# eloimoliner/BABE

Measured on AMD Instinct MI355X. Metric: audio-sec/s (blind BWE, 10 s @ 44.1 kHz clips, 35 EDM steps 2nd order), whole job, higher is better.
Workload: dtype f32

## Files before the change

### babe_amd/_cabi.py

```python
import ctypes as C


class ConvArgs(C.Structure):
    _fields_ = [
        ("in_", C.c_void_p), ("in_bs", C.c_long), ("in_cs", C.c_long),
        ("in2", C.c_void_p), ("in2_bs", C.c_long), ("in2_cs", C.c_long), ("cin_split", C.c_int),
        ("w_packed", C.c_void_p),
        ("out", C.c_void_p), ("out_bs", C.c_long), ("out_cs", C.c_long),
        ("res", C.c_void_p), ("res_bs", C.c_long), ("res_cs", C.c_long),
        ("in_scale", C.c_void_p), ("oscale", C.c_void_p),
        ("alpha", C.c_float), ("rbeta", C.c_float),
        ("B", C.c_int), ("Cin", C.c_int), ("Cout", C.c_int), ("F", C.c_int), ("T", C.c_int),
        ("KH", C.c_int), ("KW", C.c_int), ("dil", C.c_int),
        ("stat_mode", C.c_int), ("stat_cg", C.c_int), ("stat_x", C.c_void_p), ("stat_scale", C.c_void_p), ("stat_part", C.c_void_p),
        ("fbias", C.c_void_p),
    ]


class WgradArgs(C.Structure):
    _fields_ = [("x", C.c_void_p), ("x_bs", C.c_long), ("x_cs", C.c_long),
                ("x2", C.c_void_p), ("x2_bs", C.c_long), ("x2_cs", C.c_long), ("cin_split", C.c_int),
                ("g", C.c_void_p), ("g_bs", C.c_long), ("g_cs", C.c_long),
                ("B", C.c_int), ("Cin", C.c_int), ("Cout", C.c_int), ("F", C.c_int), ("T", C.c_int),
                ("KH", C.c_int), ("KW", C.c_int), ("dil", C.c_int)]
# ... 25 lines not shown
                ("oct", C.c_void_p), ("binoct", C.c_void_p), ("tw4096", C.c_void_p),
                ("nocts", C.c_int), ("binsoct", C.c_int), ("coef", C.c_void_p * 8),
                ("wg_first", C.c_void_p), ("wg_count", C.c_void_p), ("nwg", C.c_int),
                ("wg_rec", C.c_void_p), ("band_rec", C.c_void_p), ("abl", C.c_int),
                ("max_wg_count", C.c_int), ("min_log2T", C.c_int), ("max_log2T", C.c_int),
                ("sum_T", C.c_long), ("sum_M", C.c_long), ("sum_TlogT", C.c_double),
                ("kdeg", C.c_int), ("kpoly", C.c_float * 12)]


class FitCfg(C.Structure):
    _fields_ = [("mu_fc", C.c_float), ("mu_A", C.c_float), ("tol_fc", C.c_float), ("tol_A", C.c_float),
                ("fcmin", C.c_float), ("fcmax", C.c_float), ("Amin", C.c_float), ("Amax", C.c_float),
                ("max_iter", C.c_int), ("clamp_fc", C.c_int), ("clamp_A", C.c_int), ("only_negative_A", C.c_int),
                ("weighting", C.c_int), ("kernel", C.c_int)]


class EvalDesc(C.Structure):
    _fields_ = [("unet_plan", C.c_void_p), ("unet_state", C.c_void_p), ("cqt_plan", C.c_void_p), ("L", C.c_int),
                ("rff_freq", C.c_void_p), ("rff_n", C.c_int),
                ("emb_W", C.c_void_p * 3), ("emb_b", C.c_void_p * 3), ("emb_dim", C.c_int * 4),
                ("film_W", C.c_void_p), ("film_b", C.c_void_p), ("film_J", C.c_int),
                ("nfft", C.c_int), ("fs", C.c_float), ("env_inv", C.c_void_p), ("tw4096", C.c_void_p), ("K", C.c_int),
                ("fit", FitCfg), ("blind", C.c_int), ("shared", C.c_int), ("hpf", C.c_int),
                ("xi", C.c_float), ("score_mode", C.c_int), ("audio_len_norm", C.c_float)]


class DnConvArgs(C.Structure):
    _fields_ = [("in_", C.c_void_p), ("in_bs", C.c_long), ("in_cs", C.c_long), ("IH", C.c_int), ("IW", C.c_int),
                ("bias", C.c_void_p),
                ("out", C.c_void_p), ("out_bs", C.c_long), ("out_cs", C.c_long), ("out_H", C.c_int), ("out_W", C.c_int),
                ("out_hstep", C.c_int), ("out_h0", C.c_int), ("out_wstep", C.c_int), ("out_w0", C.c_int),
                ("res", C.c_void_p), ("res_bs", C.c_long), ("res_cs", C.c_long),
                ("B", C.c_int), ("Cin", C.c_int), ("Cout", C.c_int), ("OH", C.c_int), ("OW", C.c_int),
                ("KH", C.c_int), ("KW", C.c_int), ("stride", C.c_int), ("pad_t", C.c_int), ("pad_l", C.c_int),
                ("pad_mode", C.c_int), ("act", C.c_int), ("ksplit", C.c_int), ("ws", C.c_void_p)]


STRUCTS = {"babe_conv_args": ConvArgs, "babe_wgrad_args": WgradArgs, "babe_packed_conv": CPackedConv, "babe_unet_block": CBlock,
           "babe_unet_plan_desc": CPlanDesc, "babe_cqt_bands": CqtBands, "babe_fit_cfg": FitCfg, "babe_eval_desc": EvalDesc,
           "babe_dnconv_args": DnConvArgs}

_P, _L, _I, _F, _D, _S = C.c_void_p, C.c_long, C.c_int, C.c_float, C.c_double, C.c_char_p

SIGS = {
    "babe_version": (_S, []),
    "babe_last_error": (_S, []),
    "babe_conv2d_wino85_stat_slots": (_I, [C.POINTER(ConvArgs)]),
    "babe_conv_packed_size": (_L, [_I, _I, _I, _I, _I]),
    "babe_conv_pack_weights_nt": (_I, [_P, _P, _I, _I, _I, _I, _I, _I, _P]),
    "babe_conv_pack_weights_bf16": (_I, [_P, _P, _I, _I, _I, _I, _I, _I, _P]),
    "babe_conv_packed_size_bf16": (_L, [_I, _I, _I, _I, _I, _I]),
    "babe_units_size": (_L, [_I, _I, _I]),
    "babe_scale_gelu_units": (_I, [_P, _P, _P, _I, _I, _I, _I, _P]),
    "babe_conv2d_bf16_units_supported": (_I, [C.POINTER(ConvArgs)]),
    "babe_conv2d_bf16_units": (_I, [C.POINTER(ConvArgs), _P, _P]),
    "babe_conv2d_wino_supported": (_I, [C.POINTER(ConvArgs)]),
    "babe_conv_pack_weights_wino": (_I, [_P, _P, _I, _I, _I, _I, _I, _P]),
    "babe_conv_packed_size_wino": (_L, [_I, _I, _I, _I]),
    "babe_conv2d_wino4_supported": (_I, [C.POINTER(ConvArgs)]),
    "babe_conv_pack_weights_wino4": (_I, [_P, _P, _I, _I, _I, _I, _I, _P]),
    "babe_conv_packed_size_wino4": (_L, [_I, _I, _I, _I]),
    "babe_conv2d_wino45": (_I, [C.POINTER(ConvArgs), _P, _P]),
    "babe_conv2d_wino45_supported": (_I, [C.POINTER(ConvArgs)]),
    "babe_conv_pack_weights_wino45": (_I, [_P, _P, _I, _I, _I, _I, _I, _P]),
    "babe_conv_packed_size_wino45": (_L, [_I, _I, _I]),
    "babe_prof_nslots": (_I, []),
    "babe_prof_slot_name": (_S, [_I]),
    "babe_prof_enable": (_I, [_I]),
    "babe_prof_conv_slot": (_I, [_I]),
    "babe_prof_read": (_I, [_P, _P, _P, _P, _P]),
    "babe_prof_dispatch_counts": (_I, [_P, _I]),
    "babe_prof_timeline": (_L, [_P, _P, _P, _P, _P, _L]),
    "babe_prof_pending": (_L, []),
    "babe_gn_partial": (_I, [_P, _P, _I, _I, _L, _I, _P]),
    "babe_gn_stats": (_I, [_P, _P, _P, _P, _P, _L, _P, _P, _I, _I, _I, _L, _I, _F, _P]),
    "babe_gn_finalize": (_I, [_P, _P, _P, _L, _P, _P, _I, _I, _I, _L, _I, _F, _P]),
    "babe_scale_gelu_fin": (_I, [_P, _P, _P, _P, _L, _P, _P, _P, _I, _I, _I, _L, _I, _F, _P]),
    "babe_scale_gelu": (_I, [_P, _P, _P, _I, _I, _L, _P]),
    "babe_gn_bwd_partial": (_I, [_P, _P, _P, _P, _I, _I, _I, _L, _I, _P]),
    "babe_gn_bwd_apply": (_I, [_P, _P, _P, _P, _P, _P, _P, _F, _I, _I, _I, _L, _I, _F, _P]),
    "babe_gn_bwd_apply_merge": (_I, [_P, _P, _P, _P, _P, _P, _P, _F, _I, _I, _I, _L, _I, _F, _P, _P, _F, _F]),
    "babe_gn_bwd_partial_nogelu": (_I, [_P, _P, _P, _P, _I, _I, _I, _L, _I, _P]),
    "babe_gn_bwd_apply_nogelu": (_I, [_P, _P, _P, _P, _P, _P, _P, _F, _I, _I, _I, _L, _I, _F, _P]),
    "babe_resample": (_I, [_P, _L, _L, _P, _L, _L, _I, _I, _I, _I, _I, _F, _F, _P]),
    "babe_resample_res": (_I, [_P, _L, _L, _P, _L, _L, _P, _L, _L, _I, _I, _I, _I, _I, _F, _F, _P]),
    "babe_resample_sinc": (_I, [_P, _L, _P, _L, _I, _L, _L, _P, _P, _I, _I, _I, _P]),
    "babe_resample_sinc_adjoint": (_I, [_P, _L, _P, _L, _I, _L, _L, _P, _P, _I, _I, _I, _P]),
    "babe_iir_workspace": (_L, [_I, _L, _I]),
    "babe_iir_filter": (_I, [_P, _L, _P, _L, _I, _L, _P, _P, _I, _I, _I, _P, _L, _P, _L, _P]),
    "babe_decimate": (_I, [_P, _L, _P, _L, _I, _L, _L, _I, _I, _P]),
    "babe_clip_residual": (_I, [_P, _L, _P, _L, _F, _P, _L, _P, _L, _P, _I, _I, _L, _P]),
    "babe_clip_fwd": (_I, [_P, _L, _F, _P, _L, _I, _L, _P]),
    "babe_clip_adj": (_I, [_P, _L, _P, _L, _P, _L, _I, _L, _P]),
    "babe_specnorm_workspace": (_L, [_I, _I, _I]),
    "babe_specnorm_seed": (_I, [_P, _L, _I, _I, _I, _P, _L, _I, _P, _L, _P]),
    "babe_stft_mag_workspace": (_L, [_I, _I, _I]),
    "babe_stft_mag_fwd": (_I, [_P, _L, _L, _P, _I, _I, _P, _P, _I, _I, _P, _P]),
    "babe_stft_mag_vjp": (_I, [_P, _P, _P, _I, _I, _P, _L, _L, _I, _I, _P, _P, _L, _P]),
    "babe_conv_packed_size_wino85": (_L, [_I, _I, _I]),
    "babe_conv_pack_weights_wino85": (_I, [_P, _P, _I, _I, _I, _I, _I, _P]),
    "babe_conv2d_wino85_supported": (_I, [C.POINTER(ConvArgs)]),
    "babe_conv2d_wino85_preferred": (_I, [C.POINTER(ConvArgs)]),
    "babe_conv2d_wino85": (_I, [C.POINTER(ConvArgs), _P, _P]),
    "babe_conv2d_wino85_set_waves": (_I, [_I]),
    "babe_conv2d_auto": (_I, [C.POINTER(ConvArgs), C.POINTER(CPackedConv), _I, _P]),
    "babe_unet_plan_create": (_P, [C.POINTER(CPlanDesc)]),
    "babe_unet_plan_destroy": (None, [_P]),
    "babe_unet_state_create": (_P, []),
    "babe_unet_state_destroy": (None, [_P]),
    "babe_unet_workspace_bytes": (_L, [_P, _I, C.POINTER(_I)]),
    "babe_unet_fwd": (_I, [_P, _P, C.POINTER(_P), _P, _L, _I, C.POINTER(_I), _P, _L, C.POINTER(_P), _P]),
    "babe_unet_vjp": (_I, [_P, _P, C.POINTER(_P), C.POINTER(_P), _P]),
    "babe_axpby4d": (_I, [_P, _L, _L, _P, _L, _L, _I, _I, _I, _I, _F, _F, _P]),
    "babe_axpby2_4d": (_I, [_P, _L, _L, _P, _L, _L, _P, _L, _L, _I, _I, _I, _I, _F, _F, _P]),
    "babe_linear": (_I, [_P, _P, _P, _P, _I, _I, _I, _I, _P]),
    "babe_rff": (_I, [_P, _P, _P, _I, _I, _P]),
    "babe_rfft_mixed": (_I, [_P, _P, _P, _P, _P, _I, _I, _I, _I, _P, _I, _P, _I, _P, _P, _P, _I, _P]),
    "babe_fft_twiddle_transpose": (_I, [_P, _P, _P, _I, _I, _I, _I, _P]),
    "babe_cqt_band_analysis": (_I, [C.POINTER(CqtBands), _P, _P, _I, _P]),
    "babe_cqt_band_synthesis": (_I, [C.POINTER(CqtBands), _P, _P, _L, _I, _P]),
    "babe_cqt_gather": (_I, [_P, _L, _P, _P, _P, _P, _I, _I, _F, _P, _I, _P]),
    "babe_spec_scale": (_I, [_P, _P, _P, _P, _I, _I, _F, _F, _I, _P]),
    "babe_cqt_design_create": (_P, [_D, _I, _I, _I, _D]),
    "babe_cqt_design_destroy": (None, [_P]),
    "babe_cqt_design_get": (_L, [_P, _S, _P, _L]),
    "babe_cqt_plan_create": (_P, [_D, _I, _I, _I, _D]),
    "babe_cqt_plan_destroy": (None, [_P]),
    "babe_cqt_workspace_bytes": (_L, [_P, _I]),
    "babe_cqt_fwd": (_I, [_P, _P, _P, _P, _I, _P]),
    "babe_cqt_bwd": (_I, [_P, _P, _P, _P, _I, _P]),
    "babe_cqt_fwd_adjoint": (_I, [_P, _P, _P, _P, _I, _P]),
    "babe_cqt_bwd_adjoint": (_I, [_P, _P, _P, _P, _I, _P]),
    "babe_cqt_hpf": (_I, [_P, _P, _P, _P, _I, _P]),
    "babe_stft_fwd": (_I, [_P, _L, _I, _P, _P, _I, _I, _I, _P, _P]),
    "babe_spec_filter_istft": (_I, [_P, _P, _L, _P, _I, _I, _I, _P, _P]),
    "babe_ola": (_I, [_P, _P, _P, _L, _P, _L, _P, _I, _I, _I, _I, _I, _P]),
    "babe_residual_seed": (_I, [_P, _L, _P, _I, _P, _P, _L, _I, _I, _P]),
    "babe_stft_mag_stats": (_I, [_P, _P, _P, _I, _I, _I, _I, _P]),
    "babe_design_filter": (_I, [_P, _P, _I, _I, _I, _F, _I, _P]),
    "babe_filter_fit": (_I, [_P, _P, _P, _I, _I, _I, _F, _I, C.POINTER(FitCfg), _P]),
    "babe_filter_loss_grad": (_I, [_P, _L, _P, _P, _I, _I, _I, _F, _I, C.POINTER(FitCfg), _P]),
    "babe_fir_same": (_I, [_P, _L, _P, _I, _P, _L, _I, _I, _I, _P]),
    "babe_fir_sqerr_fwd": (_I, [_P, _L, _P, _L, _P, _I, _P, _P, _I, _I, _P]),
    "babe_fir_sqerr_bwd": (_I, [_P, _L, _P, _P, _I, _P, _I, _I, _P]),
    "babe_plane_bin_energy": (_I, [_P, _P, _I, _I, _I, _P]),
    "babe_lsd_num_frames": (_L, [_I, _I, _I]),
    "babe_lsd_frames": (_I, [_P, _L, _P, _L, _I, _I, _I, _I, _I, _I, _F, _P, _P, _P]),
    "babe_lincomb3": (_I, [_P, _F, _P, _F, _P, _F, _P, _L, _P]),
    "babe_add_obs_noise": (_I, [_P, _L, _P, _L, _F, _I, _L, _P]),
    "babe_mask_blend": (_I, [_P, _P, _L, _P, _P, _I, _L, _P]),
    "babe_sumsq_partial": (_I, [_P, _L, _P, _I, _I, _L, _P]),
    "babe_stft_dist_partial": (_I, [_P, _P, _P, _P, _I, _I, _I, _I, _I, _P]),
    "babe_stft_dist_grad": (_I, [_P, _P, _P, _P, _I, _P, _I, _I, _I, _I, _I, _P]),
    "babe_cos_partial": (_I, [_P, _L, _P, _L, _P, _I, _I, _L, _P]),
    "babe_residual_seed_alt": (_I, [_P, _L, _P, _L, _P, _I, _P, _P, _L, _I, _I, _I, _F, _P]),
    "babe_score_direction": (_I, [_P, _P, _P, _P, _I, _P, _F, _F, _F, _I, _I, _I, _L, _P]),
    "babe_eval_workspace_bytes": (_L, [C.POINTER(EvalDesc), _I]),
    "babe_score_eval": (_I, [C.POINTER(EvalDesc), _P, _F, _F, _F, _F, _F, _P, _P, _P, _P, _P, _P, _P, _L, _I, _P]),
    "babe_dn_conv2d": (_I, [C.POINTER(DnConvArgs), _P, _P]),
    "babe_dn_pack_weights": (_I, [_P, _P, _I, _I, _I, _I, _I, _I, _I, _P]),
    "babe_dn_packed_size": (_L, [_I, _I, _I, _I]),
    "babe_dn_upsample_add": (_I, [_P, _L, _L, _P, _L, _L, _I, _I, _I, _I, _I, _I, _I, _I, _P]),
    "babe_dn_sam_gate": (_I, [_P, _P, _P, _L, _L, _P, _L, _L, _I, _I, _L, _P]),
    "babe_dn_fill_input": (_I, [_P, _P, _P, _I, _I, _I, _I, _P]),
    "babe_dn_stft": (_I, [_P, _L, _I, _P, _I, _I, _I, _I, _P, _P]),
    "babe_dn_istft": (_I, [_P, _P, _P, _L, _I, _I, _I, _I, _I, _P, _P]),
# ... 38 lines not shown
```

### babe_amd/csrc/norm.hip

```cpp
#include "common.h"
#include "../../include/babe_hip.h"
#include "prof.h"
#include "gelu.h"
#include <cstdlib>

namespace {

using babe_gelu::gelu_f;
using babe_gelu::gelu_grad_f;

__device__ __forceinline__ void block_reduce2(double& s0, double& s1, double* sh) {
    s0 = wave_sum(s0);
    s1 = wave_sum(s1);
    const int lane = threadIdx.x & 63, wave = threadIdx.x >> 6;
    if (lane == 0) {
        sh[wave * 2] = s0;
        sh[wave * 2 + 1] = s1;
    }
    __syncthreads();
    if (threadIdx.x == 0) {
        double a = 0, b = 0;
        for (int w = 0; w < (int)(blockDim.x >> 6); ++w) {
            a += sh[w * 2];
            b += sh[w * 2 + 1];
// ... 292 lines not shown
                const float4 x0 = *reinterpret_cast<const float4*>(x + base + i);
                const float4 d0 = *reinterpret_cast<const float4*>(dadu + base + i);
                const float4 x1 = *reinterpret_cast<const float4*>(x + base + i + st);
                const float4 d1 = *reinterpret_cast<const float4*>(dadu + base + i + st);
                sc_sum += term(x0, d0);
                sc_sum += term(x1, d1);
            }
            for (; i < hi; i += st)
                sc_sum += term(*reinterpret_cast<const float4*>(x + base + i), *reinterpret_cast<const float4*>(dadu + base + i));
            s0 += (double)sc * sc_sum;
        }
    }
    block_reduce2(s0, s1, sh);
    if (threadIdx.x == 0) part[(long)bg * S + s] = s0;
}

template <bool GELU>
__global__ __launch_bounds__(256) void gn_bwd_apply_kernel(const float* __restrict__ x, const float* __restrict__ da,
                                                           const float* __restrict__ gy,
                                                           const float* __restrict__ scale,
                                                           const float* __restrict__ stats,
                                                           const double* __restrict__ part, float* __restrict__ gx,
                                                           float rbeta, int C, int G, long hw, int S, float eps,
                                                           const float* __restrict__ acc, float ca, float cb) {
    const int c = blockIdx.y, b = blockIdx.z;
    const int cg = C / G;
    const int g = c / cg;
    const long n = (long)cg * hw;
    __shared__ double S1_sh;
    if (threadIdx.x < 64) {
        double v = 0;
        for (int s = threadIdx.x; s < S; s += 64) v += part[(long)(b * G + g) * S + s];
        v = wave_sum(v);
        if (threadIdx.x == 0) S1_sh = v;
    }
    __syncthreads();
    const double S1 = S1_sh;
    const float mean = stats[(b * G + g) * 3 + 0];
    const float sd = stats[(b * G + g) * 3 + 1];
    const double se = (double)sd + eps;
    const float coef = (sd > 0.f) ? (float)(S1 * se / ((double)(n - 1) * sd * se * se)) : 0.f;
    const float sc = scale[b * C + c];
    const long base = ((long)b * C + c) * hw;
    const long nv = hw / 4;
    const float4* x4 = reinterpret_cast<const float4*>(x + base);
    const float4* d4 = reinterpret_cast<const float4*>(da + base);
    const float4* g4 = gy ? reinterpret_cast<const float4*>(gy + base) : nullptr;
    float4* o4 = reinterpret_cast<float4*>(gx + base);
    for (long i = (long)blockIdx.x * blockDim.x + threadIdx.x; i < nv; i += (long)gridDim.x * blockDim.x) {
        const float4 xv = x4[i];
        float4 dv = d4[i];
        if (GELU) {
            dv.x *= gelu_grad_f(xv.x * sc);
            dv.y *= gelu_grad_f(xv.y * sc);
            dv.z *= gelu_grad_f(xv.z * sc);
            dv.w *= gelu_grad_f(xv.w * sc);
        }
        float4 o;
        o.x = sc * dv.x - (xv.x - mean) * coef;
        o.y = sc * dv.y - (xv.y - mean) * coef;
        o.z = sc * dv.z - (xv.z - mean) * coef;
        o.w = sc * dv.w - (xv.w - mean) * coef;
        if (g4) {
            const float4 gv = g4[i];
            o.x += rbeta * gv.x;
            o.y += rbeta * gv.y;
            o.z += rbeta * gv.z;
            o.w += rbeta * gv.w;
        }
        if (acc) {
#pragma clang fp contract(off)
            const float4 av = reinterpret_cast<const float4*>(acc + base)[i];
            const float px = ca * av.x, py = ca * av.y, pz = ca * av.z, pw = ca * av.w;
            const float qx = cb * o.x, qy = cb * o.y, qz = cb * o.z, qw = cb * o.w;
            o.x = px + qx;
            o.y = py + qy;
            o.z = pz + qz;
            o.w = pw + qw;
        }
        o4[i] = o;
    }
}

}

static int abl_gn() {
    static const int v = [] { const char* e = getenv("BABE_ABL_GN"); return e ? atoi(e) : 0; }();
    return v;
}

extern "C" int babe_gn_partial(const float* x, double* part, int B, int G, long n, int S, void* stream) {
    BABE_CHECK_ARG(x && part && B > 0 && G > 0 && n > 1 && S > 0, "gn_partial: bad arguments");
    if (abl_gn() & 1) return BABE_OK;
    BABE_CHECK_ARG(n % 4 == 0, "gn_partial: group size %ld not a multiple of 4", n);
    BabeProfScope prof(BABE_SLOT_GN_STATS, 4.0 * B * G * (double)n, 0, 0, stream);
    hipLaunchKernelGGL(gn_partial_kernel<false>, dim3(S, B * G), dim3(256), 0, (hipStream_t)stream, x, part, n, S,
                       (int*)nullptr, (const float*)nullptr, (const float*)nullptr, 0L, (float*)nullptr, (float*)nullptr, 0, 1, 0.f);
    BABE_LAUNCH_CHECK();
    return BABE_OK;
}

extern "C" int babe_gn_stats(const float* x, double* part, int* ticket, const float* gamma, const float* film, long film_bs,
                             float* stats, float* scale, int B, int C, int G, long n, int S, float eps, void* stream) {
    BABE_CHECK_ARG(x && part && ticket && gamma && film && stats && scale && B > 0 && G > 0 && n > 1 && S > 0, "gn_stats: bad arguments");
    BABE_CHECK_ARG(n % 4 == 0 && G <= 64 && C % G == 0, "gn_stats: n=%ld C=%d G=%d unsupported", n, C, G);
    BabeProfScope prof(BABE_SLOT_GN_STATS, 4.0 * B * G * (double)n, 0, 0, stream);
    hipLaunchKernelGGL(gn_partial_kernel<true>, dim3(S, B * G), dim3(256), 0, (hipStream_t)stream, x, part, n, S, ticket, gamma,
                       film, film_bs, stats, scale, C, G, eps);
    BABE_LAUNCH_CHECK();
    return BABE_OK;
}

extern "C" int babe_gn_finalize(const double* part, const float* gamma, const float* film, long film_bs, float* stats,
                                float* scale, int B, int C, int G, long n, int S, float eps, void* stream) {
    BABE_CHECK_ARG(part && gamma && film && stats && scale, "gn_finalize: null pointer");
    BABE_CHECK_ARG(G <= 64 && C % G == 0, "gn_finalize: C=%d G=%d unsupported", C, G);
    BabeProfScope prof(BABE_SLOT_GN_STATS, 0, 0, 0, stream);
    hipLaunchKernelGGL(gn_finalize_kernel, dim3(B), dim3(256), 0, (hipStream_t)stream, part, gamma, film, film_bs,
                       stats, scale, C, G, n, S, eps);
    BABE_LAUNCH_CHECK();
    return BABE_OK;
}

extern "C" int babe_scale_gelu(const float* x, const float* scale, float* a, int B, int C, long hw, void* stream) {
    BABE_CHECK_ARG(x && scale && a && B > 0 && C > 0 && hw > 0, "scale_gelu: bad arguments");
    BABE_CHECK_ARG(hw % 4 == 0, "scale_gelu: plane size %ld not a multiple of 4", hw);
    BabeProfScope prof(BABE_SLOT_SCALE_GELU, 8.0 * B * C * (double)hw, 0, 0, stream);
    int bx = cdiv(hw / 4, 256 * 4);
    if (bx < 1) bx = 1;
    if (bx > 64) bx = 64;
    hipLaunchKernelGGL(scale_gelu_kernel, dim3(bx, C, B), dim3(256), 0, (hipStream_t)stream, x, scale, a, C, hw);
    BABE_LAUNCH_CHECK();
    return BABE_OK;
}

extern "C" int babe_scale_gelu_fin(const float* x, const double* part, const float* gamma, const float* film, long film_bs,
                                   float* stats, float* scale, float* a, int B, int C, int G, long hw, int S, float eps,
                                   void* stream) {
    BABE_CHECK_ARG(x && part && gamma && film && stats && scale && a && B > 0 && C > 0 && hw > 0 && S > 0, "scale_gelu_fin: bad arguments");
    BABE_CHECK_ARG(hw % 4 == 0 && G <= 64 && C % G == 0, "scale_gelu_fin: hw=%ld C=%d G=%d unsupported", hw, C, G);
    BabeProfScope prof(BABE_SLOT_SCALE_GELU, 8.0 * B * C * (double)hw, 0, 0, stream);
    int bx = cdiv(hw / 4, 256 * 4);
    if (bx < 1) bx = 1;
    if (bx > 64) bx = 64;
    const long n = (long)(C / G) * hw;
    hipLaunchKernelGGL(scale_gelu_fin_kernel, dim3(bx, C, B), dim3(256), 0, (hipStream_t)stream, x, part, gamma, film, film_bs,
                       stats, scale, a, C, G, hw, n, S, eps);
    BABE_LAUNCH_CHECK();
    return BABE_OK;
}

extern "C" long babe_units_size(int C, int F, int T) { return (long)(C / 8) * F * 4 * (T / 4 + 1); }

extern "C" int babe_scale_gelu_units(const float* x, const float* scale, void* au, int B, int C, int F, int T,
                                     void* stream) {
    BABE_CHECK_ARG(x && scale && au && B > 0 && C > 0 && F > 0 && T > 0, "scale_gelu_units: bad arguments");
    BABE_CHECK_ARG(T % 4 == 0 && C % 8 == 0, "scale_gelu_units: T=%d C=%d unsupported (need T %% 4 == 0, C %% 8 == 0)", T, C);
    BABE_CHECK_ARG(((uintptr_t)x & 15) == 0 && ((uintptr_t)au & 15) == 0, "scale_gelu_units: unaligned pointer");
    BabeProfScope prof(BABE_SLOT_SCALE_GELU, 6.0 * B * C * (double)F * T, 0, 0, stream);
    int bx = cdiv((long)F * (T / 4), 256 * 2);
    if (bx < 1) bx = 1;
    if (bx > 256) bx = 256;
    hipLaunchKernelGGL(scale_gelu_units_kernel, dim3(bx, C / 8, B), dim3(256), 0, (hipStream_t)stream, x, scale,
                       (bf16x8_n*)au, C, F, T);
    BABE_LAUNCH_CHECK();
    return BABE_OK;
}

extern "C" int babe_gn_bwd_partial(const float* x, const float* da, const float* scale, double* part, int B, int C,
                                   int G, long hw, int S, void* stream) {
    BABE_CHECK_ARG(x && da && scale && part, "gn_bwd_partial: null pointer");
    BABE_CHECK_ARG(hw % 4 == 0 && C % G == 0, "gn_bwd_partial: hw=%ld C=%d G=%d unsupported", hw, C, G);
    if (abl_gn() & 2) return BABE_OK;
    BabeProfScope prof(BABE_SLOT_GN_BWD_PARTIAL, 8.0 * B * C * (double)hw, 0, 0, stream);
    hipLaunchKernelGGL(gn_bwd_partial_kernel<true>, dim3(S, B * G), dim3(256), 0, (hipStream_t)stream, x, da, scale,
                       part, C, G, hw, S);
    BABE_LAUNCH_CHECK();
    return BABE_OK;
}

extern "C" int babe_gn_bwd_partial_nogelu(const float* x, const float* da, const float* scale, double* part, int B, int C,
                                          int G, long hw, int S, void* stream) {
    BABE_CHECK_ARG(x && da && scale && part, "gn_bwd_partial_nogelu: null pointer");
    BABE_CHECK_ARG(hw % 4 == 0 && C % G == 0, "gn_bwd_partial_nogelu: hw=%ld C=%d G=%d unsupported", hw, C, G);
    BabeProfScope prof(BABE_SLOT_GN_BWD_PARTIAL, 8.0 * B * C * (double)hw, 0, 0, stream);
    hipLaunchKernelGGL(gn_bwd_partial_kernel<false>, dim3(S, B * G), dim3(256), 0, (hipStream_t)stream, x, da, scale,
                       part, C, G, hw, S);
    BABE_LAUNCH_CHECK();
    return BABE_OK;
}

static int gn_bwd_apply_launch(bool gelu, const float* acc, float ca, float cb, const float* x, const float* da, const float* gy, const float* scale,
                                 const float* stats, const double* part, float* gx, float rbeta, int B, int C, int G,
                                 long hw, int S, float eps, void* stream) {
    BABE_CHECK_ARG(x && da && scale && stats && part && gx, "gn_bwd_apply: null pointer");
    BABE_CHECK_ARG(hw % 4 == 0 && C % G == 0, "gn_bwd_apply: hw=%ld C=%d G=%d unsupported", hw, C, G);
    BabeProfScope prof(BABE_SLOT_GN_BWD_APPLY, ((gy ? 16.0 : 12.0) + (acc ? 4.0 : 0.0)) * B * C * (double)hw, 0, 0, stream);
    int bx = cdiv(hw / 4, 256 * 4);
    if (bx < 1) bx = 1;
    if (bx > 64) bx = 64;
    if (gelu)
        hipLaunchKernelGGL(gn_bwd_apply_kernel<true>, dim3(bx, C, B), dim3(256), 0, (hipStream_t)stream, x, da, gy, scale, stats,
                           part, gx, rbeta, C, G, hw, S, eps, acc, ca, cb);
    else
        hipLaunchKernelGGL(gn_bwd_apply_kernel<false>, dim3(bx, C, B), dim3(256), 0, (hipStream_t)stream, x, da, gy, scale, stats,
                           part, gx, rbeta, C, G, hw, S, eps, acc, ca, cb);
    BABE_LAUNCH_CHECK();
    return BABE_OK;
}

extern "C" int babe_gn_bwd_apply(const float* x, const float* da, const float* gy, const float* scale,
                                 const float* stats, const double* part, float* gx, float rbeta, int B, int C, int G,
                                 long hw, int S, float eps, void* stream) {
    return gn_bwd_apply_launch(true, nullptr, 0.f, 0.f, x, da, gy, scale, stats, part, gx, rbeta, B, C, G, hw, S, eps, stream);
}

extern "C" int babe_gn_bwd_apply_nogelu(const float* x, const float* da, const float* gy, const float* scale,
                                        const float* stats, const double* part, float* gx, float rbeta, int B, int C, int G,
                                        long hw, int S, float eps, void* stream) {
    return gn_bwd_apply_launch(false, nullptr, 0.f, 0.f, x, da, gy, scale, stats, part, gx, rbeta, B, C, G, hw, S, eps, stream);
}

extern "C" int babe_gn_bwd_apply_merge(const float* x, const float* da, const float* gy, const float* scale,
                                 const float* stats, const double* part, float* gx, float rbeta, int B, int C, int G,
                                 long hw, int S, float eps, void* stream, const float* acc, float ca, float cb) {
    BABE_CHECK_ARG(acc && ((uintptr_t)acc & 15) == 0, "gn_bwd_apply_merge: acc must be a 16-byte aligned dense tensor");
    return gn_bwd_apply_launch(true, acc, ca, cb, x, da, gy, scale, stats, part, gx, rbeta, B, C, G, hw, S, eps, stream);
}
```

### include/babe_hip.h

```cpp
#ifndef BABE_HIP_H
#define BABE_HIP_H
#ifdef __cplusplus
extern "C" {
#endif

const char* babe_version(void);
const char* babe_last_error(void);

typedef struct { float* p; long bs; long cs; } babe_view;

typedef struct {
    const float* in;  long in_bs,  in_cs;
    const float* in2; long in2_bs, in2_cs; int cin_split;
    const float* w_packed;
    float* out;       long out_bs, out_cs;
    const float* res; long res_bs, res_cs;
    const float* in_scale;
    const float* oscale;
    float alpha, rbeta;
    int B, Cin, Cout, F, T, KH, KW, dil;
    int stat_mode, stat_cg;
    const float* stat_x; const float* stat_scale; double* stat_part;
    const float* fbias;
} babe_conv_args;
int babe_conv2d_wino85_stat_slots(const babe_conv_args* a);
int babe_conv2d(const babe_conv_args* a, void* stream);
int babe_conv_pack_weights(const float* w, float* dst, int Cout, int Cin, int KH, int KW,
                           int transpose_flip, void* stream);
long babe_conv_packed_size(int Cout, int Cin, int KH, int KW, int transpose_flip);
int babe_conv2d_nt(const babe_conv_args* a, int nt, void* stream);
int babe_conv_pack_weights_nt(const float* w, float* dst, int Cout, int Cin, int KH, int KW, int transpose_flip, int nt,
                              void* stream);
int babe_conv2d_bf16(const babe_conv_args* a, const void* w_bf16, int splits, void* stream);
int babe_conv_pack_weights_bf16(const float* w, void* dst, int Cout, int Cin, int KH, int KW, int transpose_flip,
                                int splits, void* stream);
long babe_conv_packed_size_bf16(int Cout, int Cin, int KH, int KW, int transpose_flip, int splits);
long babe_units_size(int C, int F, int T);
int babe_scale_gelu_units(const float* x, const float* scale, void* units, int B, int C, int F, int T, void* stream);
int babe_conv2d_bf16_units_supported(const babe_conv_args* a);
int babe_conv2d_bf16_units(const babe_conv_args* a, const void* w_bf16, void* stream);
int babe_conv2d_wino(const babe_conv_args* a, const float* w_wino, void* stream);
int babe_conv2d_wino_supported(const babe_conv_args* a);
int babe_conv_pack_weights_wino(const float* w, float* dst, int Cout, int Cin, int KH, int KW, int transpose_flip,
                                void* stream);
long babe_conv_packed_size_wino(int Cout, int Cin, int KH, int transpose_flip);
int babe_conv2d_wino4(const babe_conv_args* a, const float* w_wino4, void* stream);
int babe_conv2d_wino4_supported(const babe_conv_args* a);
int babe_conv_pack_weights_wino4(const float* w, float* dst, int Cout, int Cin, int KH, int KW, int transpose_flip,
                                 void* stream);
long babe_conv_packed_size_wino4(int Cout, int Cin, int KH, int transpose_flip);
int babe_conv2d_wino45(const babe_conv_args* a, const float* w_wino45, void* stream);
int babe_conv2d_wino45_supported(const babe_conv_args* a);
int babe_conv2d_wino45_preferred(const babe_conv_args* a);
int babe_conv_pack_weights_wino45(const float* w, float* dst, int Cout, int Cin, int KH, int KW, int transpose_flip,
                                  void* stream);
long babe_conv_packed_size_wino45(int Cout, int Cin, int transpose_flip);
int babe_conv2d_fewco(const babe_conv_args* a, const float* w, int transpose_flip, void* stream);
int babe_conv2d_fewco_supported(const babe_conv_args* a);
int babe_prof_nslots(void);
const char* babe_prof_slot_name(int slot);
int babe_prof_enable(int on);
int babe_prof_conv_slot(int slot);
int babe_prof_read(double* ms, double* bytes, double* flops, double* exec_flops, long* launches);
int babe_prof_dispatch_counts(long* counts, int reset);
long babe_prof_timeline(double* t0_ms, double* t1_ms, int* slot, int* lane, double* flops, long cap);
long babe_prof_pending(void);

int babe_gn_partial(const float* x, double* part, int B, int G, long n_per_group, int S, void* stream);
int babe_gn_stats(const float* x, double* part, int* ticket, const float* gamma, const float* film, long film_bs,
                  float* stats, float* scale, int B, int C, int G, long n_per_group, int S, float eps, void* stream);
int babe_gn_finalize(const double* part, const float* gamma, const float* film, long film_bs,
                     float* stats, float* scale, int B, int C, int G, long n_per_group, int S,
                     float eps, void* stream);
int babe_scale_gelu_fin(const float* x, const double* part, const float* gamma, const float* film, long film_bs, float* stats,
                        float* scale, float* a, int B, int C, int G, long hw, int S, float eps, void* stream);
int babe_scale_gelu(const float* x, const float* scale, float* a, int B, int C, long hw, void* stream);
int babe_gn_bwd_partial(const float* x, const float* da, const float* scale, double* part,
                        int B, int C, int G, long hw, int S, void* stream);
int babe_gn_bwd_apply(const float* x, const float* da, const float* gy, const float* scale,
                      const float* stats, const double* part, float* gx, float rbeta,
                      int B, int C, int G, long hw, int S, float eps, void* stream);
int babe_gn_bwd_apply_merge(const float* x, const float* da, const float* gy, const float* scale,
                            const float* stats, const double* part, float* gx, float rbeta,
                            int B, int C, int G, long hw, int S, float eps, void* stream,
                            const float* acc, float ca, float cb);
int babe_gn_bwd_partial_nogelu(const float* x, const float* da, const float* scale, double* part, int B, int C, int G, long hw,
                               int S, void* stream);
int babe_gn_bwd_apply_nogelu(const float* x, const float* da, const float* gy, const float* scale, const float* stats,
                             const double* part, float* gx, float rbeta, int B, int C, int G, long hw, int S, float eps,
                             void* stream);

int babe_resample(const float* in, long in_bs, long in_cs, float* out, long out_bs, long out_cs,
                  int B, int C, int F, int T, int mode, float alpha, float beta, void* stream);
int babe_resample_res(const float* in, long in_bs, long in_cs, const float* res, long res_bs, long res_cs, float* out,
                      long out_bs, long out_cs, int B, int C, int F, int T, int mode, float alpha, float beta, void* stream);

int babe_resample_sinc(const float* x, long x_bs, float* out, long out_bs, int B, long L_in, long L_out, const float* kernel,
                       const int* krange, int orig, int new_, int width, void* stream);
int babe_resample_sinc_adjoint(const float* g, long g_bs, float* out, long out_bs, int B, long L_in, long L_out,
                               const float* kernel, const int* krange, int orig, int new_, int width, void* stream);

long babe_iir_workspace(int B, long L, int order);
int babe_iir_filter(const float* x, long x_bs, float* y, long y_bs, int B, long L, const float* b, const float* a, int order,
                    int clamp, int adjoint, unsigned char* mask, long mask_bs, void* workspace, long workspace_bytes, void* stream);
int babe_decimate(const float* in, long in_bs, float* out, long out_bs, int B, long L_full, long L_dec, int factor, int adjoint,
                  void* stream);

int babe_clip_residual(const float* x, long x_bs, const float* y, long y_bs, float c, float* r, long r_bs, unsigned char* mask,
                       long mask_bs, double* part, int nblk, int B, long L, void* stream);
int babe_clip_fwd(const float* x, long x_bs, float c, float* out, long out_bs, int B, long L, void* stream);
int babe_clip_adj(const float* g, long g_bs, const unsigned char* mask, long mask_bs, float* out, long out_bs, int B, long L,
                  void* stream);
long babe_specnorm_workspace(int B, int rows, int cols);
int babe_specnorm_seed(const float* r, long r_bs, int rows, int cols, int iters, float* out, long out_bs, int B, void* workspace,
                       long workspace_bytes, void* stream);
long babe_stft_mag_workspace(int B, int frames, int win);
int babe_stft_mag_fwd(const float* x, long x_bs, long L, const float* window, int win, int hop, float* spec, float* mag, int B,
                      int frames, const float* tw4096, void* stream);
int babe_stft_mag_vjp(const float* G, const float* spec, const float* window, int win, int hop, float* gx, long gx_bs, long L,
                      int B, int frames, const float* tw4096, void* workspace, long workspace_bytes, void* stream);

long babe_conv_packed_size_wino85(int Cout, int Cin, int transpose_flip);
int babe_conv_pack_weights_wino85(const float* w, float* dst, int Cout, int Cin, int KH, int KW, int transpose_flip, void* stream);
int babe_conv2d_wino85_supported(const babe_conv_args* a);
int babe_conv2d_wino85_preferred(const babe_conv_args* a);
int babe_conv2d_wino85(const babe_conv_args* a, const float* w_wino85, void* stream);
int babe_conv2d_wino85_set_waves(int waves);

typedef struct {
    int Cout, Cin, KH, KW, nt, splits;
    const void *fwd, *bwd;
    const float *fwd_wino, *bwd_wino, *fwd_wino4, *bwd_wino4, *fwd_wino45, *bwd_wino45;
    const float* w_raw;
    const float *fwd_wino85, *bwd_wino85;
} babe_packed_conv;
int babe_conv2d_auto(babe_conv_args* a, const babe_packed_conv* pc, int transpose, void* stream);
typedef struct {
    int N, nd, k53;
    babe_packed_conv proj_in, res_conv, proj_out, H[8];
    const float* gamma[8];
    int film_aff[8], film_gate[8];
    const float *fb_proj_in, *fb_res_conv;
} babe_unet_block;
typedef struct {
    int nocts, bpo;
    int Ns[8];
    babe_unet_block init_blk[8], main_blk[8], up_out[8], up_blk[8], mid_blk, mid_out;
    babe_packed_conv pyr_conv[8];
} babe_unet_plan_desc;
void* babe_unet_plan_create(const babe_unet_plan_desc* desc);
void babe_unet_plan_destroy(void* plan);
void* babe_unet_state_create(void);
void babe_unet_state_destroy(void* state);
long babe_unet_workspace_bytes(const void* plan, int B, const int* T_oct);
int babe_unet_fwd(const void* plan, void* state, const float* const* C_in, const float* film, long film_bs, int B,
                  const int* T_oct, void* workspace, long workspace_bytes, float* const* outs, void* stream);
int babe_unet_vjp(const void* plan, void* state, const float* const* gouts, float* const* gC, void* stream);

int babe_axpby4d(const float* in, long in_bs, long in_cs, float* out, long out_bs, long out_cs,
                 int B, int C, int F, int T, float alpha, float beta, void* stream);
int babe_fill4d(float* out, long out_bs, long out_cs, int B, int C, int F, int T, float value, void* stream);
int babe_axpby2_4d(const float* x, long x_bs, long x_cs, const float* y, long y_bs, long y_cs, float* out, long out_bs,
                   long out_cs, int B, int C, int F, int T, float alpha, float beta, void* stream);

int babe_linear(const float* x, const float* W, const float* bias, float* out, int B, int K, int J,
                int relu, void* stream);
int babe_rff(const float* cnoise, const float* freq, float* out, int B, int R, void* stream);

int babe_rfft_mixed(const float* x_in, float* spec_out, const float* spec_in, float* x_out, float* work, int B, int N1,
                    int N2, int K2, const int* rad1, int nrad1, const int* rad2, int nrad2, const float* w1, const float* w2,
                    const float* tw, int direction, void* stream);
int babe_fft_twiddle_transpose(const float* in, float* out, const float* tw, int B, int N1, int N2,
                               int adjoint, void* stream);
// ... 192 lines not shown
```

Before: 2.470.

## Add alternate GroupNorm kernel forms with load rings and specialized apply variants

```diff
diff --git a/babe_amd/_cabi.py b/babe_amd/_cabi.py
--- a/babe_amd/_cabi.py
+++ b/babe_amd/_cabi.py
@@ -131,6 +131,8 @@
     "babe_gn_bwd_apply_merge": (_I, [_P, _P, _P, _P, _P, _P, _P, _F, _I, _I, _I, _L, _I, _F, _P, _P, _F, _F]),
     "babe_gn_bwd_partial_nogelu": (_I, [_P, _P, _P, _P, _I, _I, _I, _L, _I, _P]),
     "babe_gn_bwd_apply_nogelu": (_I, [_P, _P, _P, _P, _P, _P, _P, _F, _I, _I, _I, _L, _I, _F, _P]),
+    "babe_norm_set_form": (_I, [_I]),
+    "babe_norm_get_form": (_I, []),
     "babe_resample": (_I, [_P, _L, _L, _P, _L, _L, _I, _I, _I, _I, _I, _F, _F, _P]),
     "babe_resample_res": (_I, [_P, _L, _L, _P, _L, _L, _P, _L, _L, _I, _I, _I, _I, _I, _F, _F, _P]),
     "babe_resample_sinc": (_I, [_P, _L, _P, _L, _I, _L, _L, _P, _P, _I, _I, _I, _P]),
diff --git a/babe_amd/csrc/norm.hip b/babe_amd/csrc/norm.hip
--- a/babe_amd/csrc/norm.hip
+++ b/babe_amd/csrc/norm.hip
@@ -398,7 +398,341 @@
     }
 }
 
-}
+namespace f1 {
+
+__device__ __forceinline__ double sum4(const float4 v) {
+#pragma clang fp contract(off)
+    return (((double)v.x + (double)v.y) + (double)v.z) + (double)v.w;
+}
+__device__ __forceinline__ double sq4(const float4 v) {
+#pragma clang fp contract(off)
+    double a = (double)v.y * (double)v.y;
+    a = __builtin_fma((double)v.x, (double)v.x, a);
+    a = __builtin_fma((double)v.z, (double)v.z, a);
+    return __builtin_fma((double)v.w, (double)v.w, a);
+}
+
+template <int NT, int PAIR>
+__device__ __forceinline__ void slot_sums(const double* __restrict__ pg, int S, double& t0, double& t1) {
+    t0 = 0;
+    t1 = 0;
+    for (int q = threadIdx.x; q < S; q += NT * 4) {
+        double a[4], c[4];
+#pragma unroll
+        for (int k = 0; k < 4; ++k) {
+            const int qq = q + NT * k < S ? q + NT * k : S - 1;
+            a[k] = pg[(long)qq * PAIR];
+            c[k] = PAIR == 2 ? pg[(long)qq * PAIR + PAIR - 1] : 0.0;
+        }
+#pragma unroll
+        for (int k = 0; k < 4; ++k)
+            if (q + NT * k < S) {
+                t0 += a[k];
+                if (PAIR == 2) t1 += c[k];
+            }
+    }
+}
+
+__global__ __launch_bounds__(256) void gn_partial_kernel(const float* __restrict__ x, double* __restrict__ part, long n, int S) {
+    __shared__ double sh[8];
+    const int s = blockIdx.x;
+    const long bg = blockIdx.y;
+    const long chunk = ((n / 4 + S - 1) / S) * 4;
+    const long beg = (long)s * chunk;
+    long end = beg + chunk;
+    if (end > n) end = n;
+    const float* p = x + bg * n;
+    double s0 = 0, s1 = 0;
+    if (beg < end) {
+#pragma clang fp contract(off)
+        const long nv = (end - beg) / 4;
+        const float4* p4 = reinterpret_cast<const float4*>(p + beg);
+        long i = threadIdx.x;
+        for (; i + 7 * 256L < nv; i += 8 * 256L) {
+            float4 v[8];
+#pragma unroll
+            for (int k = 0; k < 8; ++k) v[k] = p4[i + k * 256L];
+            s0 += ((sum4(v[0]) + sum4(v[1])) + sum4(v[2])) + sum4(v[3]);
+            s1 += ((sq4(v[0]) + sq4(v[1])) + sq4(v[2])) + sq4(v[3]);
+            s0 += ((sum4(v[4]) + sum4(v[5])) + sum4(v[6])) + sum4(v[7]);
+            s1 += ((sq4(v[4]) + sq4(v[5])) + sq4(v[6])) + sq4(v[7]);
+        }
+        for (; i + 3 * 256L < nv; i += 4 * 256L) {
+            const float4 v0 = p4[i], v1 = p4[i + 256L], v2 = p4[i + 2 * 256L], v3 = p4[i + 3 * 256L];
+            s0 += ((sum4(v0) + sum4(v1)) + sum4(v2)) + sum4(v3);
+            s1 += ((sq4(v0) + sq4(v1)) + sq4(v2)) + sq4(v3);
+        }
+        for (; i < nv; i += 256L) {
+            const float4 v = p4[i];
+            s0 += sum4(v);
+            s1 += sq4(v);
+        }
+        for (long j = beg + nv * 4 + threadIdx.x; j < end; j += 256L) {
+            const double v = p[j];
+            s0 += v;
+            s1 = __builtin_fma(v, v, s1);
+        }
+    }
+    block_reduce2(s0, s1, sh);
+    if (threadIdx.x == 0) {
+        part[(bg * S + s) * 2] = s0;
+        part[(bg * S + s) * 2 + 1] = s1;
+    }
+}
+
+__device__ __forceinline__ float4 scale_gelu4(float4 v, const float sc) {
+#pragma clang fp contract(off)
+    v.x = gelu_f(v.x * sc);
+    v.y = gelu_f(v.y * sc);
+    v.z = gelu_f(v.z * sc);
+    v.w = gelu_f(v.w * sc);
+    return v;
+}
+
+constexpr int kGeluLoads = 4;
+
+template <int NLD, typename L>
+struct Ring {
+    L buf[NLD];
+    template <typename Load>
+    __device__ __forceinline__ void first(long i0, long gs, long nv, Load&& load) {
+#pragma unroll
+        for (int d = 0; d < NLD; ++d) {
+            const long j = i0 + d * gs;
+            buf[d] = load(j < nv ? j : nv - 1);
+        }
+    }
+    template <typename Load, typename Use>
+    __device__ __forceinline__ void run(long i0, long gs, long nv, Load&& load, Use&& use) {
+        for (long i = i0; i < nv; i += NLD * gs) {
+#pragma unroll
+            for (int d = 0; d < NLD; ++d) {
+                const long j = i + d * gs;
+                if (j < nv) use(j, buf[d]);
+                if (j + NLD * gs < nv) buf[d] = load(j + NLD * gs);
+            }
+        }
+    }
+};
+
+__global__ __launch_bounds__(256) void scale_gelu_kernel(const float* __restrict__ x, const float* __restrict__ scale,
+                                                         float* __restrict__ a, int C, long hw) {
+    const int c = blockIdx.y, b = blockIdx.z;
+    const long base = ((long)b * C + c) * hw;
+    const long nv = hw / 4;
+    const float4* x4 = reinterpret_cast<const float4*>(x + base);
+    float4* a4 = reinterpret_cast<float4*>(a + base);
+    const long i0 = (long)blockIdx.x * 256 + threadIdx.x, gs = (long)gridDim.x * 256;
+    auto load = [&](long j) { return x4[j]; };
+    Ring<kGeluLoads, float4> ring;
+    ring.first(i0, gs, nv, load);
+    const float sc = scale[b * C + c];
+    ring.run(i0, gs, nv, load, [&](long j, const float4 v) { a4[j] = scale_gelu4(v, sc); });
+}
+
+__global__ __launch_bounds__(256) void scale_gelu_fin_kernel(const float* __restrict__ x, const double* __restrict__ part,
+                                                             const float* __restrict__ gamma, const float* __restrict__ film,
+                                                             long film_bs, float* __restrict__ stats, float* __restrict__ scale,
+                                                             float* __restrict__ a, int C, int G, long hw, long n, int S,
+                                                             float eps) {
+    __shared__ float sc_sh;
+    __shared__ double red_sh[512];
+    const int c = blockIdx.y, b = blockIdx.z;
+    const int cg = C / G, g = c / cg;
+    const long base = ((long)b * C + c) * hw;
+    const long nv = hw / 4;
+    const float4* x4 = reinterpret_cast<const float4*>(x + base);
+    float4* a4 = reinterpret_cast<float4*>(a + base);
+    const long i0 = (long)blockIdx.x * 256 + threadIdx.x, gs = (long)gridDim.x * 256;
+    auto load = [&](long j) { return x4[j]; };
+    Ring<kGeluLoads, float4> ring;
+    ring.first(i0, gs, nv, load);
+    {
+        double t0, t1;
+        slot_sums<256, 2>(part + (long)(b * G + g) * S * 2, S, t0, t1);
+        red_sh[threadIdx.x * 2] = t0;
+        red_sh[threadIdx.x * 2 + 1] = t1;
+    }
+    __syncthreads();
+    if (threadIdx.x < 32) {
+        double t0 = 0, t1 = 0;
+#pragma unroll
+        for (int j = 0; j < 8; ++j) {
+            t0 += red_sh[(threadIdx.x + 32 * j) * 2];
+            t1 += red_sh[(threadIdx.x + 32 * j) * 2 + 1];
+        }
+#pragma unroll
+        for (int o = 16; o >= 1; o >>= 1) {
+            t0 += __shfl_xor(t0, o, 32);
+            t1 += __shfl_xor(t1, o, 32);
+        }
+        if (threadIdx.x == 0) {
+            const double mean = t0 / (double)n;
+            double var = (t1 - (double)n * mean * mean) / (double)(n - 1);
+            if (var < 0) var = 0;
+            const float sd = (float)sqrt(var);
+            const float r = 1.f / (sd + eps);
+            const float scv = gamma[c] * (film[(long)b * film_bs + c] + 1.f) * r;
+            sc_sh = scv;
+            if (blockIdx.x == 0) {
+                scale[b * C + c] = scv;
+                if (c == g * cg) {
+                    stats[(b * G + g) * 3 + 0] = (float)mean;
+                    stats[(b * G + g) * 3 + 1] = sd;
+                    stats[(b * G + g) * 3 + 2] = r;
+                }
+            }
+        }
+    }
+    __syncthreads();
+    const float sc = sc_sh;
+    ring.run(i0, gs, nv, load, [&](long j, const float4 v) { a4[j] = scale_gelu4(v, sc); });
+}
+
+template <bool GELU>
+__device__ __forceinline__ double bwd_term(const float4 xv, float4 dv, const float sc) {
+#pragma clang fp contract(off)
+    if (GELU) {
+        dv.x = dv.x * gelu_grad_f(xv.x * sc);
+        dv.y = dv.y * gelu_grad_f(xv.y * sc);
+        dv.z = dv.z * gelu_grad_f(xv.z * sc);
+        dv.w = dv.w * gelu_grad_f(xv.w * sc);
+    }
+    double t = (double)dv.y * (double)xv.y;
+    t = __builtin_fma((double)dv.x, (double)xv.x, t);
+    t = __builtin_fma((double)dv.z, (double)xv.z, t);
+    return __builtin_fma((double)dv.w, (double)xv.w, t);
+}
+
+template <bool GELU>
+__global__ __launch_bounds__(256) void gn_bwd_partial_kernel(const float* __restrict__ x, const float* __restrict__ dadu,
+                                                             const float* __restrict__ scale,
+                                                             double* __restrict__ part, int C, int G, long hw, int S) {
+    __shared__ double sh[8];
+    const int s = blockIdx.x;
+    const int bg = blockIdx.y;
+    const int b = bg / G, g = bg % G;
+    const int cg = C / G;
+    const long n = (long)cg * hw;
+    const long chunk = ((n / 4 + S - 1) / S) * 4;
+    const long beg = (long)s * chunk;
+    long end = beg + chunk;
+    if (end > n) end = n;
+    const long base = ((long)b * C + (long)g * cg) * hw;
+    double s0 = 0, s1 = 0;
+    if (beg < end) {
+#pragma clang fp contract(off)
+        const int c_lo = (int)(beg / hw), c_hi = (int)((end - 1) / hw);
+        for (int cl = c_lo; cl <= c_hi; ++cl) {
+            const long lo = beg > (long)cl * hw ? beg : (long)cl * hw;
+            const long hi = end < (long)(cl + 1) * hw ? end : (long)(cl + 1) * hw;
+            const float sc = scale[b * C + g * cg + cl];
+            double sc_sum = 0;
+            const long st = 256L * 4;
+            long i = lo + (long)threadIdx.x * 4;
+            for (; i + 3 * st < hi; i += 4 * st) {
+                float4 xv[4], dv[4];
+#pragma unroll
+                for (int k = 0; k < 4; ++k) {
+                    xv[k] = *reinterpret_cast<const float4*>(x + base + i + k * st);
+                    dv[k] = *reinterpret_cast<const float4*>(dadu + base + i + k * st);
+                }
+                __builtin_amdgcn_sched_barrier(0);
+#pragma unroll
+                for (int k = 0; k < 4; ++k) sc_sum += bwd_term<GELU>(xv[k], dv[k], sc);
+            }
+            for (; i < hi; i += st)
+                sc_sum += bwd_term<GELU>(*reinterpret_cast<const float4*>(x + base + i), *reinterpret_cast<const float4*>(dadu + base + i), sc);
+            s0 = __builtin_fma((double)sc, sc_sum, s0);
+        }
+    }
+    block_reduce2(s0, s1, sh);
+    if (threadIdx.x == 0) part[(long)bg * S + s] = s0;
+}
+
+struct ApplyLoads { float4 x, d, gy, acc; };
+
+template <bool GELU, bool HAS_GY, bool HAS_ACC>
+__global__ __launch_bounds__(256) void gn_bwd_apply_kernel(const float* __restrict__ x, const float* __restrict__ da,
+                                                           const float* __restrict__ gy,
+                                                           const float* __restrict__ scale,
+                                                           const float* __restrict__ stats,
+                                                           const double* __restrict__ part, float* __restrict__ gx,
+                                                           float rbeta, int C, int G, long hw, int S, float eps,
+                                                           const float* __restrict__ acc, float ca, float cb) {
+    constexpr int NLD = (HAS_GY || HAS_ACC) ? 2 : 3;
+    const int c = blockIdx.y, b = blockIdx.z;
+    const int cg = C / G;
+    const int g = c / cg;
+    const long n = (long)cg * hw;
+    const long base = ((long)b * C + c) * hw;
+    const long nv = hw / 4;
+    const float4* x4 = reinterpret_cast<const float4*>(x + base);
+    const float4* d4 = reinterpret_cast<const float4*>(da + base);
+    const float4* g4 = reinterpret_cast<const float4*>((HAS_GY ? gy : x) + base);
+    const float4* c4 = reinterpret_cast<const float4*>((HAS_ACC ? acc : x) + base);
+    float4* o4 = reinterpret_cast<float4*>(gx + base);
+    const long i0 = (long)blockIdx.x * 256 + threadIdx.x, gs = (long)gridDim.x * 256;
+    auto load = [&](long j) {
+        ApplyLoads l;
+        l.x = x4[j];
+        l.d = d4[j];
+        if (HAS_GY) l.gy = g4[j];
+        if (HAS_ACC) l.acc = c4[j];
+        return l;
+    };
+    Ring<NLD, ApplyLoads> ring;
+    ring.first(i0, gs, nv, load);
+    __shared__ double S1_sh;
+    if (threadIdx.x < 64) {
+        double v, unused;
+        slot_sums<64, 1>(part + (long)(b * G + g) * S, S, v, unused);
+        v = wave_sum(v);
+        if (threadIdx.x == 0) S1_sh = v;
+    }
+    __syncthreads();
+    const double S1 = S1_sh;
+    const float mean = stats[(b * G + g) * 3 + 0];
+    const float sd = stats[(b * G + g) * 3 + 1];
+    const double se = (double)sd + eps;
+    const float coef = (sd > 0.f) ? (float)(S1 * se / ((double)(n - 1) * sd * se * se)) : 0.f;
+    const float sc = scale[b * C + c];
+    auto one = [&](float xe, float de, float ge, float ae) {
+#pragma clang fp contract(off)
+        if (GELU) de = de * gelu_grad_f(xe * sc);
+        float o = __builtin_fmaf(sc, de, -((xe - mean) * coef));
+        if (HAS_GY) o = __builtin_fmaf(rbeta, ge, o);
+        if (HAS_ACC) {
+            const float p = ca * ae, q = cb * o;
+            o = p + q;
+        }
+        return o;
+    };
+    ring.run(i0, gs, nv, load, [&](long j, const ApplyLoads& l) {
+        float4 o;
+        o.x = one(l.x.x, l.d.x, l.gy.x, l.acc.x);
+        o.y = one(l.x.y, l.d.y, l.gy.y, l.acc.y);
+        o.z = one(l.x.z, l.d.z, l.gy.z, l.acc.z);
+        o.w = one(l.x.w, l.d.w, l.gy.w, l.acc.w);
+        o4[j] = o;
+    });
+}
+
+}
+
+}
+
+static std::atomic<int>& norm_form() {
+    static std::atomic<int> v{[] { const char* e = getenv("BABE_NORM_FORM"); return (e && atoi(e) == 0) ? 0 : 1; }()};
+    return v;
+}
+extern "C" int babe_norm_set_form(int form) {
+    BABE_CHECK_ARG(form == 0 || form == 1, "norm_set_form: 0 or 1 (got %d)", form);
+    norm_form().store(form, std::memory_order_relaxed);
+    return BABE_OK;
+}
+extern "C" int babe_norm_get_form(void) { return norm_form().load(std::memory_order_relaxed); }
+static bool form1() { return norm_form().load(std::memory_order_relaxed) == 1; }
 
 static int abl_gn() {
     static const int v = [] { const char* e = getenv("BABE_ABL_GN"); return e ? atoi(e) : 0; }();
@@ -410,8 +744,11 @@
     if (abl_gn() & 1) return BABE_OK;
     BABE_CHECK_ARG(n % 4 == 0, "gn_partial: group size %ld not a multiple of 4", n);
     BabeProfScope prof(BABE_SLOT_GN_STATS, 4.0 * B * G * (double)n, 0, 0, stream);
-    hipLaunchKernelGGL(gn_partial_kernel<false>, dim3(S, B * G), dim3(256), 0, (hipStream_t)stream, x, part, n, S,
-                       (int*)nullptr, (const float*)nullptr, (const float*)nullptr, 0L, (float*)nullptr, (float*)nullptr, 0, 1, 0.f);
+    if (form1())
+        hipLaunchKernelGGL(f1::gn_partial_kernel, dim3(S, B * G), dim3(256), 0, (hipStream_t)stream, x, part, n, S);
+    else
+        hipLaunchKernelGGL(gn_partial_kernel<false>, dim3(S, B * G), dim3(256), 0, (hipStream_t)stream, x, part, n, S,
+                           (int*)nullptr, (const float*)nullptr, (const float*)nullptr, 0L, (float*)nullptr, (float*)nullptr, 0, 1, 0.f);
     BABE_LAUNCH_CHECK();
     return BABE_OK;
 }
@@ -445,7 +782,10 @@
     int bx = cdiv(hw / 4, 256 * 4);
     if (bx < 1) bx = 1;
     if (bx > 64) bx = 64;
-    hipLaunchKernelGGL(scale_gelu_kernel, dim3(bx, C, B), dim3(256), 0, (hipStream_t)stream, x, scale, a, C, hw);
+    if (form1())
+        hipLaunchKernelGGL(f1::scale_gelu_kernel, dim3(bx, C, B), dim3(256), 0, (hipStream_t)stream, x, scale, a, C, hw);
+    else
+        hipLaunchKernelGGL(scale_gelu_kernel, dim3(bx, C, B), dim3(256), 0, (hipStream_t)stream, x, scale, a, C, hw);
     BABE_LAUNCH_CHECK();
     return BABE_OK;
 }
@@ -460,8 +800,12 @@
     if (bx < 1) bx = 1;
     if (bx > 64) bx = 64;
     const long n = (long)(C / G) * hw;
-    hipLaunchKernelGGL(scale_gelu_fin_kernel, dim3(bx, C, B), dim3(256), 0, (hipStream_t)stream, x, part, gamma, film, film_bs,
-                       stats, scale, a, C, G, hw, n, S, eps);
+    if (form1())
+        hipLaunchKernelGGL(f1::scale_gelu_fin_kernel, dim3(bx, C, B), dim3(256), 0, (hipStream_t)stream, x, part, gamma, film, film_bs,
+                           stats, scale, a, C, G, hw, n, S, eps);
+    else
+        hipLaunchKernelGGL(scale_gelu_fin_kernel, dim3(bx, C, B), dim3(256), 0, (hipStream_t)stream, x, part, gamma, film, film_bs,
+                           stats, scale, a, C, G, hw, n, S, eps);
     BABE_LAUNCH_CHECK();
     return BABE_OK;
 }
@@ -489,8 +833,12 @@
     BABE_CHECK_ARG(hw % 4 == 0 && C % G == 0, "gn_bwd_partial: hw=%ld C=%d G=%d unsupported", hw, C, G);
     if (abl_gn() & 2) return BABE_OK;
     BabeProfScope prof(BABE_SLOT_GN_BWD_PARTIAL, 8.0 * B * C * (double)hw, 0, 0, stream);
-    hipLaunchKernelGGL(gn_bwd_partial_kernel<true>, dim3(S, B * G), dim3(256), 0, (hipStream_t)stream, x, da, scale,
-                       part, C, G, hw, S);
+    if (form1())
+        hipLaunchKernelGGL(f1::gn_bwd_partial_kernel<true>, dim3(S, B * G), dim3(256), 0, (hipStream_t)stream, x, da, scale,
+                           part, C, G, hw, S);
+    else
+        hipLaunchKernelGGL(gn_bwd_partial_kernel<true>, dim3(S, B * G), dim3(256), 0, (hipStream_t)stream, x, da, scale,
+                           part, C, G, hw, S);
     BABE_LAUNCH_CHECK();
     return BABE_OK;
 }
@@ -500,8 +848,12 @@
     BABE_CHECK_ARG(x && da && scale && part, "gn_bwd_partial_nogelu: null pointer");
     BABE_CHECK_ARG(hw % 4 == 0 && C % G == 0, "gn_bwd_partial_nogelu: hw=%ld C=%d G=%d unsupported", hw, C, G);
     BabeProfScope prof(BABE_SLOT_GN_BWD_PARTIAL, 8.0 * B * C * (double)hw, 0, 0, stream);
-    hipLaunchKernelGGL(gn_bwd_partial_kernel<false>, dim3(S, B * G), dim3(256), 0, (hipStream_t)stream, x, da, scale,
-                       part, C, G, hw, S);
+    if (form1())
+        hipLaunchKernelGGL(f1::gn_bwd_partial_kernel<false>, dim3(S, B * G), dim3(256), 0, (hipStream_t)stream, x, da, scale,
+                           part, C, G, hw, S);
+    else
+        hipLaunchKernelGGL(gn_bwd_partial_kernel<false>, dim3(S, B * G), dim3(256), 0, (hipStream_t)stream, x, da, scale,
+                           part, C, G, hw, S);
     BABE_LAUNCH_CHECK();
     return BABE_OK;
 }
@@ -515,7 +867,16 @@
     int bx = cdiv(hw / 4, 256 * 4);
     if (bx < 1) bx = 1;
     if (bx > 64) bx = 64;
-    if (gelu)
+    if (form1()) {
+        using K = void (*)(const float*, const float*, const float*, const float*, const float*, const double*, float*, float, int,
+                           int, long, int, float, const float*, float, float);
+        static const K tab[8] = {f1::gn_bwd_apply_kernel<false, false, false>, f1::gn_bwd_apply_kernel<false, false, true>,
+                                 f1::gn_bwd_apply_kernel<false, true, false>,  f1::gn_bwd_apply_kernel<false, true, true>,
+                                 f1::gn_bwd_apply_kernel<true, false, false>,  f1::gn_bwd_apply_kernel<true, false, true>,
+                                 f1::gn_bwd_apply_kernel<true, true, false>,   f1::gn_bwd_apply_kernel<true, true, true>};
+        hipLaunchKernelGGL(tab[(gelu ? 4 : 0) + (gy ? 2 : 0) + (acc ? 1 : 0)], dim3(bx, C, B), dim3(256), 0, (hipStream_t)stream, x, da,
+                           gy, scale, stats, part, gx, rbeta, C, G, hw, S, eps, acc, ca, cb);
+    } else if (gelu)
         hipLaunchKernelGGL(gn_bwd_apply_kernel<true>, dim3(bx, C, B), dim3(256), 0, (hipStream_t)stream, x, da, gy, scale, stats,
                            part, gx, rbeta, C, G, hw, S, eps, acc, ca, cb);
     else
diff --git a/include/babe_hip.h b/include/babe_hip.h
--- a/include/babe_hip.h
+++ b/include/babe_hip.h
@@ -89,6 +89,8 @@
 int babe_gn_bwd_apply_nogelu(const float* x, const float* da, const float* gy, const float* scale, const float* stats,
                              const double* part, float* gx, float rbeta, int B, int C, int G, long hw, int S, float eps,
                              void* stream);
+int babe_norm_set_form(int form);
+int babe_norm_get_form(void);
 
 int babe_resample(const float* in, long in_bs, long in_cs, float* out, long out_bs, long out_cs,
                   int B, int C, int F, int T, int mode, float alpha, float beta, void* stream);
```

Result: no change. 2.473 (median of 6 runs) (+0.1%).
